# francesco-cal98/multimodal-idbn

Measured on AMD Instinct MI355X. Metric: CD-1 updates/sec (batch 64, 10000<->1500 RBM), higher is better.
Workload: dtype f32; 1 GPU; BASELINE configs[1] layer 1: RBM 10000<->1500 train_epoch, CD-1, batch 64 per GPU, fp32 master weights, lr 0.1 wd 1e-4 mom 0.5; global_batch=64, parallelism=dp1, arithmetic=bf16x3 split MFMA (fp32-exact products)

## Files before the change

include/imdbn_engine.h:

```cpp
#ifndef IMDBN_ENGINE_H
#define IMDBN_ENGINE_H

#include <stddef.h>
#include <stdint.h>

#ifdef __cplusplus
extern "C" {
#endif

#define IMDBN_ABI_VERSION 4

#define IMDBN_E_INVALID   (-1)
#define IMDBN_E_WORKSPACE (-2)
#define IMDBN_E_RNG       (-3)
#define IMDBN_E_NODEVICE  (-4)
#define IMDBN_E_UNSUPPORTED (-5)

#define IMDBN_PARITY_F32 0
#define IMDBN_FAST_BF16  1

#define IMDBN_RNG_PHILOX 0
#define IMDBN_RNG_REPLAY 1

#define IMDBN_MAX_GROUPS 4
// ... 52 lines not shown
    int32_t sample_h;
    int32_t sample_v;
    int32_t reclamp_negative;
    const float* next_data;
    int64_t ld_next;
    int32_t next_slot;
    int32_t data_slot;
    int32_t data_binary;
    int32_t next_binary;
    float*  fwd_out;
    int64_t ld_fwd;
} imdbn_cd_opts;

int    imdbn_version(void);
int    imdbn_last_error(char* buf, size_t n);
int    imdbn_device_info(int* cu_count, char* arch, size_t n);
size_t imdbn_ws_bytes(int V, int H, int B);
int    imdbn_set_tuning(int ksplit_up, int ksplit_down);
int    imdbn_set_option(const char* name, int value);
typedef struct imdbn_options imdbn_options;
imdbn_options* imdbn_options_create(void);
void   imdbn_options_destroy(imdbn_options* o);
int    imdbn_options_set(imdbn_options* o, const char* name, int value);
int    imdbn_use_options(const imdbn_options* o);
int    imdbn_profile_enable(int on);
int    imdbn_profile_read(double* total_ms, int* launches);
int    imdbn_debug_stamps(long long* out, int n);
int    imdbn_debug_ws_offset(int V, int H, int B, const char* name, size_t* offset);
enum { IMDBN_ROUTE_UP_FUSED = 0, IMDBN_ROUTE_UP_STREAM_BITS = 1, IMDBN_ROUTE_UP_STREAM_REAL = 2, IMDBN_ROUTE_UP_PARTIAL4 = 3,
       IMDBN_ROUTE_UP_PARTIAL = 4 };
enum { IMDBN_ROUTE_DOWN_K2_STREAM = 0, IMDBN_ROUTE_DOWN_FUSED = 1, IMDBN_ROUTE_DOWN_CHUNKS2 = 2, IMDBN_ROUTE_DOWN_CHUNKS4 = 3,
       IMDBN_ROUTE_DOWN_TILED = 4 };
int    imdbn_debug_last_route(int route[5]);

int imdbn_rng_advance(uint64_t* dev_offset, uint64_t n, imdbn_stream_t stream);

int imdbn_rbm_prop_up(const imdbn_rbm_desc* d, const float* v, int64_t ldv, int B, float T,
                      imdbn_rng* rng, float* out_prob, int64_t ldo, float* out_sample, int64_t lds,
                      void* ws, size_t ws_bytes, imdbn_stream_t stream);

int imdbn_rbm_forward(const imdbn_rbm_desc* d, const float* v, int64_t ldv, int B, int data_binary,
                      float* out_prob, int64_t ldo, void* ws, size_t ws_bytes, imdbn_stream_t stream);

int imdbn_rbm_free_energy(const imdbn_rbm_desc* d, const float* v, int64_t ldv, int B, float* out_F,
                          void* ws, size_t ws_bytes, imdbn_stream_t stream);

int imdbn_rbm_ais(const imdbn_rbm_desc* d, int M, int K, const float* betas, const float* base_vis_bias, imdbn_rng* rng,
                  double* logw, float* out_v, int64_t ldo, void* ws, size_t ws_bytes, imdbn_stream_t stream);

int imdbn_rbm_ais_groups(const imdbn_rbm_desc* d, int M, int K, const float* betas, const float* base_vis_bias, imdbn_rng* rng,
                         double* logw, float* out_v, int64_t ldo, void* ws, size_t ws_bytes, imdbn_stream_t stream);

int imdbn_rbm_reverse_ais(const imdbn_rbm_desc* d, const float* v, int64_t ldv, int R, int K, const float* betas,
                          const float* base_vis_bias, imdbn_rng* rng, double* logw, float* out_v, int64_t ldo,
                          void* ws, size_t ws_bytes, imdbn_stream_t stream);

int imdbn_rows_logmeanexp(const double* logw, int N, int M, double* out_lme, double* out_ess, imdbn_stream_t stream);

int imdbn_rbm_label_loglik(const imdbn_rbm_desc* d, const float* z, int64_t ldz, int N, int Dz, int K, const int32_t* gt,
                           double* out_joint, double* out_marg, void* ws, size_t ws_bytes, imdbn_stream_t stream);

int imdbn_rbm_label_step(const imdbn_rbm_desc* d, const float* z, int64_t ldz, int N, int Dz, int K, const int32_t* gt,
                         const imdbn_cd_opts* o, double* out_logp, float* scratch, void* ws, size_t ws_bytes, imdbn_stream_t stream);

int imdbn_rbm_pseudo_loglik(const imdbn_rbm_desc* d, const float* v, int64_t ldv, int N, double* out_pll, float* out_site, int64_t lds,
                            void* ws, size_t ws_bytes, imdbn_stream_t stream);
// ... 158 lines not shown
```

multimodal-idbn_amd/csrc/engine.hip:

```cpp
#include <hip/hip_runtime.h>

#include <algorithm>
#include <atomic>
#include <climits>
#include <cstdarg>
#include <cstdio>
#include <cstring>
#include <dlfcn.h>
#include <mutex>
#include <new>
#include <vector>

#include "../../include/imdbn_engine.h"
#include "kernels_ew.hpp"
#include "kernels_gemm.hpp"
#include "kernels_chain.hpp"
#include "kernels_stream.hpp"
#include "kernels_trace.hpp"
#include "kernels_knn.hpp"
#include "kernels_energy.hpp"
#include "kernels_metrics.hpp"
#include "kernels_ais.hpp"
#include "kernels_reverse_ais.hpp"
#include "kernels_bound.hpp"
// ... 480 lines not shown
    g_prof.calls = 0;
    return 0;
}

int imdbn_debug_stamps(long long* out, int n) {
    if (!out || n <= 0 || n > 4096 * 8) return fail(IMDBN_E_INVALID, "imdbn_debug_stamps: bad buffer");
    HIPCHK(hipDeviceSynchronize());
    HIPCHK(hipMemcpyFromSymbol(out, HIP_SYMBOL(g_stamps), sizeof(long long) * (size_t)n, 0, hipMemcpyDeviceToHost));
    static const std::vector<long long> zeros(4096 * 8, 0);
    HIPCHK(hipMemcpyToSymbol(HIP_SYMBOL(g_stamps), zeros.data(), sizeof(long long) * zeros.size(), 0, hipMemcpyHostToDevice));
    return 0;
}

int imdbn_debug_ws_offset(int V, int H, int B, const char* name, size_t* offset) {
    if (V <= 0 || H <= 0 || B <= 0 || !name || !offset) return fail(IMDBN_E_INVALID, "debug_ws_offset: bad argument");
    char* fake = reinterpret_cast<char*>((uintptr_t)1 << 30);
    const Layout L = make_layout(V, H, B, fake);
    const void* p = nullptr;
    if (!strcmp(name, "vis_bits0")) p = L.vis_bits[0]; else if (!strcmp(name, "vis_bits1")) p = L.vis_bits[1];
    else if (!strcmp(name, "hid_bits")) p = L.hid_bits; else if (!strcmp(name, "vis_tr0")) p = L.vis_tr[0];
    else if (!strcmp(name, "vis_tr1")) p = L.vis_tr[1]; else if (!strcmp(name, "hid_tr0")) p = L.hid_tr[0];
    else if (!strcmp(name, "hid_tr1")) p = L.hid_tr[1]; else if (!strcmp(name, "cs_hpos")) p = L.cs_hpos;
    else if (!strcmp(name, "cs_hneg")) p = L.cs_hneg; else if (!strcmp(name, "cs_vpos")) p = L.cs_vpos;
    else if (!strcmp(name, "cs_vneg")) p = L.cs_vneg; else if (!strcmp(name, "flags")) p = L.flags;
    else if (!strcmp(name, "partial")) p = L.partial; else if (!strcmp(name, "vis_rm1")) p = L.vis_rm[1];
    else return fail(IMDBN_E_INVALID, "debug_ws_offset: unknown buffer %s", name);
    *offset = (size_t)((const char*)p - fake);
    return 0;
}

int imdbn_debug_last_route(int route[5]) {
    if (!route) return fail(IMDBN_E_INVALID, "imdbn_debug_last_route: null buffer");
    route[0] = t_route.up; route[1] = t_route.up_general; route[2] = t_route.down; route[3] = t_route.down_general; route[4] = t_route.down_groups;
    return 0;
}

int imdbn_profile_read(double* total_ms, int* launches) {
    double tot = 0.0;
    for (size_t i = 0; i + 1 < g_prof.used; i += 2) {
        HIPCHK(hipEventSynchronize(g_prof.ev[i + 1]));
        float ms = 0.f;
        HIPCHK(hipEventElapsedTime(&ms, g_prof.ev[i], g_prof.ev[i + 1]));
        tot += ms;
    }
    if (total_ms) *total_ms = tot;
    if (launches) *launches = (int)(g_prof.used / 2);
    g_prof.used = 0;
    return 0;
}

__global__ void rng_advance_kernel(unsigned long long* p, unsigned long long n) { *p += n; }
int imdbn_rng_advance(uint64_t* dev_offset, uint64_t n, imdbn_stream_t stream) {
    if (!dev_offset) return fail(IMDBN_E_INVALID, "rng_advance: null counter");
    hipLaunchKernelGGL(rng_advance_kernel, dim3(1), dim3(1), 0, S(stream), (unsigned long long*)dev_offset, (unsigned long long)n);
    HIPCHK(hipGetLastError());
    return 0;
}

int imdbn_rbm_prop_up(const imdbn_rbm_desc* d, const float* v, int64_t ldv, int B, float T, imdbn_rng* rng,
                      float* out_prob, int64_t ldo, float* out_sample, int64_t lds, void* ws, size_t ws_bytes,
                      imdbn_stream_t stream) {
    CHK(check_desc(d, false));
    if (!v || !out_prob || ldv < d->V || ldo < d->H) return fail(IMDBN_E_INVALID, "prop_up: bad tensor argument");
    Ctx c(d, rng, S(stream));
    CHK(setup(c, B, ws, ws_bytes));
    FinishArgs f = new_finish();
// ... 485 lines not shown
    const Layout& L = c.L;
    const char* fb = fake + L.fb_off;
    if (((head_stride | planes_stride) & 255) || ((((uintptr_t)head) | ((uintptr_t)planes)) & 255) || planes_stride < L.fb_bytes ||
        head_stride < (size_t)((const char*)L.vis_tr[0] - fb))
        return fail(IMDBN_E_INVALID, "apply_factors: the gathered blocks must be 256-B aligned and at least %zu bytes apart", L.fb_bytes);
    auto at_h = [&](const void* layout_ptr, int rk) { return (const char*)head + ((const char*)layout_ptr - fb) + (size_t)rk * head_stride; };
    auto at_v = [&](const void* layout_ptr, int rk) { return (const char*)planes + ((const char*)layout_ptr - fb) + (size_t)rk * planes_stride; };
    AssocPlanesArgs f;
    memset(&f, 0, sizeof(f));
    f.W = d->W; f.Wm = d->W_m; f.ldw = d->ldw; f.V = L.V; f.H = L.H;
    f.vpos_terms = c.nw == 1 ? 1 : 0; f.vneg_terms = 1;
    f.vts = (int64_t)L.V * L.Bp; f.hts = (int64_t)L.H * L.Bp; f.Bp = L.Bp;
    f.lr = o->lr; f.mom = o->momentum; f.wd = o->weight_decay; f.n = (float)global_B;
    BiasArgs b = make_bias(c, o, o->sparsity != 0, (float)global_B, loss_out);
    b.hpos = (const float*)at_h(L.cs_hpos, 0); b.hneg = (const float*)at_h(L.cs_hneg, 0);
    b.vpos = (const float*)at_h(L.cs_vpos, 0); b.vneg = (const float*)at_h(L.cs_vneg, 0);
    b.loss_part = (const float*)at_h(L.loss_part, 0);
    b.R = n_ranks; b.rs = (int64_t)(head_stride / 4);
    BiasArgs bz;
    memset(&bz, 0, sizeof(bz));
    const int tpb = c.r.tpb, brows = k3_bias_rows(L);
    ProfBracket prof;
    CHK(prof.begin(c.s, true));
    if (n_ranks >= tune().min_rank_loop && !tune().no_rank_loop && f.vneg_terms == 1) {
        f.vpos = (const bf16_t*)at_v(L.vis_tr[0], 0); f.vpos_flag = (const int*)at_h(L.flags, 0);
        f.hpos = (const bf16_t*)at_h(L.hid_tr[0], 0);
        f.vneg = (const bf16_t*)at_v(L.vis_tr[1], 0); f.hneg = (const bf16_t*)at_h(L.hid_tr[1], 0);
        RankLoopArgs rl{n_ranks, (int64_t)(head_stride / 2), (int64_t)(planes_stride / 2)};
        const bool acc = tpb <= 4 && !tune().no_rank_acc;
        const auto k = c.ht == 3 ? (acc ? assoc_update_planes_ranks<3, true> : assoc_update_planes_ranks<3, false>)
                                 : (acc ? assoc_update_planes_ranks<1, true> : assoc_update_planes_ranks<1, false>);
        hipLaunchKernelGGL(k, k3_grid(c, brows), dim3(256), 0, c.s, f, rl, tpb, b, brows);
        HIPCHK(hipGetLastError());
        return prof.end(c.s);
    }
    for (int rk = 0; rk < n_ranks; ++rk) {
        f.vpos = (const bf16_t*)at_v(L.vis_tr[0], rk); f.vpos_flag = (const int*)at_h(L.flags, rk);
        f.hpos = (const bf16_t*)at_h(L.hid_tr[0], rk);
        f.vneg = (const bf16_t*)at_v(L.vis_tr[1], rk); f.hneg = (const bf16_t*)at_h(L.hid_tr[1], rk);
        const int br = (rk == n_ranks - 1) ? brows : 0;
        CHK(launch_k3_planes(c, 0, f, k3_pass(rk, n_ranks), br ? b : bz, br));
    }
    return prof.end(c.s);
}

int imdbn_rbm_apply_factors(const imdbn_rbm_desc* d, const void* gathered, int n_ranks, size_t rank_stride, int rows_per_rank,
                            int global_B, const imdbn_cd_opts* o, float* loss_out, imdbn_stream_t stream) {
    return apply_factors_impl(d, gathered, rank_stride, gathered, rank_stride, n_ranks, rows_per_rank, global_B, o, loss_out, stream);
}

int imdbn_rbm_apply_factors_wire(const imdbn_rbm_desc* d, const void* wire, size_t wire_stride, const void* planes, size_t planes_stride,
                                 int n_ranks, int rows_per_rank, int global_B, const imdbn_cd_opts* o, float* loss_out, imdbn_stream_t stream) {
    return apply_factors_impl(d, wire, wire_stride, planes, planes_stride, n_ranks, rows_per_rank, global_B, o, loss_out, stream);
}

int imdbn_rbm_apply_wire(const imdbn_rbm_desc* d, const void* wire, size_t wire_stride, int n_ranks, int rows_per_rank, int global_B,
                         int binary_data, void* planes, size_t planes_stride, const imdbn_cd_opts* o, float* loss_out, imdbn_stream_t stream) {
    CHK(check_desc(d, true));
    CHK(imdbn_rbm_unpack_factors(d->V, d->H, rows_per_rank, binary_data, wire, wire_stride, n_ranks, planes, planes_stride, 1, stream));
    return apply_factors_impl(d, wire, wire_stride, planes, planes_stride, n_ranks, rows_per_rank, global_B, o, loss_out, stream);
}

int imdbn_rbm_apply_delta(const imdbn_rbm_desc* d, const float* packed, int global_B, const imdbn_cd_opts* o,
                          float* loss_out, imdbn_stream_t stream) {
    CHK(check_desc(d, true));
    if (!packed || !o || global_B <= 0) return fail(IMDBN_E_INVALID, "apply_delta: bad argument");
// ... 739 lines not shown
```

multimodal-idbn_amd/csrc/host_layout.hpp:

```cpp
#pragma once

struct Tuning {
    int ks_up = 0, ks_down = 0;
    int no_fast_k3 = 0;
    int no_fast_k1 = 0;
    int no_fused_up = 0;
    int k4_rows = 0;
    int no_rank_loop = 0;
    int no_chain_kernel = 0;
    int no_rank_acc = 0;
    int min_rank_loop = 2;
    int no_prefetch = 0;
    int no_bits = 0;
    int down_tr = 0;
    int no_k1s = 0;
    int k1s_ks = 0;
    int no_k2s = 0;
    int k2s_tr = 0;
    int no_k1s_real = 0;
    int no_adaptive = 0;
    int k1s_lds_pad = 0;
    int no_chain_pair = 0;
    int no_down_tiled = 0;
    int no_down_chunks = 0;
    int k1s_force_na = 0;
};
Tuning g_defaults;
thread_local const Tuning* t_bound = nullptr;
inline const Tuning& tune() { return t_bound ? *t_bound : g_defaults; }
int g_dbg = 0;

enum OptKind { OPT_SET, OPT_FLAG, OPT_CLAMP, OPT_CHECKED };
struct Opt { const char* name; int Tuning::*knob; OptKind kind = OPT_SET; int lo = 0, hi = 0, step = 1; };
const Opt g_opts[] = {
    {"ksplit_up", &Tuning::ks_up, OPT_CLAMP, 0, INT_MAX}, {"ksplit_down", &Tuning::ks_down, OPT_CLAMP, 0, INT_MAX},
    {"k1s_ks", &Tuning::k1s_ks, OPT_CLAMP, 0, INT_MAX}, {"k1s_lds_pad", &Tuning::k1s_lds_pad, OPT_CLAMP, 0, 64 * 1024},
    {"down_rows", &Tuning::down_tr, OPT_CHECKED, 4, 32, 4}, {"k2s_rows", &Tuning::k2s_tr, OPT_CHECKED, 8, 48, 8},
    {"chain_rows", &Tuning::k4_rows, OPT_CHECKED, 0, 16, 1},
    {"generic_k3", &Tuning::no_fast_k3, OPT_FLAG}, {"generic_k1", &Tuning::no_fast_k1, OPT_FLAG}, {"no_fused_up", &Tuning::no_fused_up, OPT_FLAG},
    {"no_rank_loop", &Tuning::no_rank_loop}, {"no_rank_acc", &Tuning::no_rank_acc}, {"min_rank_loop", &Tuning::min_rank_loop},
    {"no_chain_kernel", &Tuning::no_chain_kernel}, {"no_chain_pair", &Tuning::no_chain_pair}, {"no_bits", &Tuning::no_bits},
    {"no_prefetch", &Tuning::no_prefetch}, {"no_adaptive", &Tuning::no_adaptive}, {"k1s_force_na", &Tuning::k1s_force_na},
    {"no_k1s", &Tuning::no_k1s}, {"no_k1s_real", &Tuning::no_k1s_real}, {"no_k2s", &Tuning::no_k2s},
    {"no_down_chunks", &Tuning::no_down_chunks}, {"no_down_tiled", &Tuning::no_down_tiled},
};

int set_opt(Tuning& t, const char* name, int value) {
    if (!name) return fail(IMDBN_E_INVALID, "null option name");
    if (!strcmp(name, "dbg")) { g_dbg = value; return 0; }
    for (const Opt& o : g_opts) {
        if (strcmp(name, o.name)) continue;
        if (o.kind == OPT_CHECKED && value != 0 && (value < o.lo || value > o.hi || value % o.step)) {
            if (o.step > 1) return fail(IMDBN_E_INVALID, "%s must be 0 or a multiple of %d in [%d, %d]", o.name, o.step, o.lo, o.hi);
            return fail(IMDBN_E_INVALID, "%s must be in [%d, %d]", o.name, o.lo, o.hi);
        }
        t.*o.knob = o.kind == OPT_FLAG ? (value != 0) : (o.kind == OPT_CLAMP ? std::max(o.lo, std::min(value, o.hi)) : value);
        return 0;
    }
    return fail(IMDBN_E_INVALID, "unknown option %s", name);
}

inline int rup(int x, int m) { return (x + m - 1) / m * m; }
inline int cdiv(int a, int b) { return (a + b - 1) / b; }

struct Split { int ks; int kchunk; };
Split plan_split(int Kpad, int n_tiles, int m_blocks, int forced, int cap) {
    int ks = forced;
    if (ks <= 0) {
        const int target = 768;
        ks = std::max(1, (int)((double)target / (double)(n_tiles * m_blocks) + 0.5));
    }
    ks = std::min(ks, cap);
    ks = std::min(ks, cdiv(Kpad, 64));
    ks = std::max(ks, 1);
    const int kchunk = rup(cdiv(Kpad, ks), 64);
    return {cdiv(Kpad, kchunk), kchunk};
}
// ... 153 lines not shown
    bool neg_rm;
    bool prefetch;
    bool next_on_k1;
    bool rides;
    bool adaptive_ok;
    bool adaptive_next;
    int tpb;
    int cd_k2_blocks;

    Up up(const OpIn& in, bool logits_only) const {
        if (up_fused) return Up::fused;
        if (!k1s || logits_only) return Up::partial;
        if (in.bits && (in.binary == 1 || in.binary == 2)) return Up::stream_bits;
        return (in.rm && k1s_real && (in.binary == 0 || (in.binary == 3 && in.bits && in.flag))) ? Up::stream_real : Up::partial;
    }
    bool data_bits(int data_binary) const { return k1s && data_binary != IMDBN_DATA_REAL; }
    bool data_needs_rm(int data_binary) const { return !(k1s && data_binary == IMDBN_DATA_BINARY); }
};

Route make_route(const imdbn_rbm_desc* d, const Layout& L) {
    const Tuning& t = tune();
    Route r{};
    r.vec4 = vec4_rows(d);
    r.up_fused = L.Vpad <= 1024 && !t.no_fused_up;
    r.k1s = r.vec4 && !t.no_k1s && !r.up_fused;
    r.k1s_real = r.k1s && !t.no_k1s_real;
    r.k2s = r.vec4 && !t.no_k2s;
    r.k2s_cd = r.k2s && !t.no_bits;
    r.vbits = d->n_groups == 0 && (r.k2s_cd || L.down_tr % 8 == 0);
    r.neg_rm = !(r.vbits && r.k1s);
    r.prefetch = r.vec4 && !t.no_prefetch;
    r.next_on_k1 = r.k2s_cd && r.vbits && r.k1s;
    r.rides = !r.k2s_cd || r.next_on_k1;
    r.tpb = std::max(1, cdiv(cdiv(L.H, 128) * cdiv(L.V, 128), std::max(cu_count(), 1)));
    r.adaptive_ok = L.k1s_kchunk <= 2048 && 2 * r.tpb * L.P <= 256 && cdiv(cdiv(L.V, 128), r.tpb) <= L.k1s_tiles * L.k1s_ks;
    r.adaptive_next = r.rides && !t.no_adaptive && r.k1s_real && r.adaptive_ok;
    r.cd_k2_blocks = cdiv(L.Vpad, r.k2s_cd ? L.k2s_tr : L.down_tr);
    return r;
}
```

multimodal-idbn_amd/csrc/host_update.hpp:

```cpp
#pragma once

struct Prof {
    bool on = false;
    std::vector<hipEvent_t> ev;
    size_t used = 0;
    unsigned calls = 0;
} g_prof;
struct ProfBracket {
    bool on = false;
    int begin(hipStream_t s, bool wanted) {
        on = wanted && g_prof.on && (g_prof.calls++ % 8 == 3) && g_prof.used + 2 <= g_prof.ev.size();
        if (on) HIPCHK(hipEventRecord(g_prof.ev[g_prof.used], s));
        return 0;
    }
    int end(hipStream_t s) {
        if (on) { HIPCHK(hipEventRecord(g_prof.ev[g_prof.used + 1], s)); g_prof.used += 2; }
        return 0;
    }
};

BiasArgs make_bias(Ctx& c, const imdbn_cd_opts* o, bool sparsity, float n, float* loss_out) {
    const Layout& L = c.L;
    BiasArgs b;
    memset(&b, 0, sizeof(b));
    b.hid_bias = c.d->hid_bias; b.hb_m = c.d->hb_m; b.H = L.H; b.hpos = L.cs_hpos; b.hneg = L.cs_hneg;
    b.vis_bias = c.d->vis_bias; b.vb_m = c.d->vb_m; b.V = L.V; b.vpos = L.cs_vpos; b.vneg = L.cs_vneg;
    b.P = L.P; b.lr = o->lr; b.mom = o->momentum; b.n = n;
    b.sparsity = sparsity ? 1 : 0; b.target = o->sparsity_target;
    b.loss_part = L.loss_part; b.n_loss = n_loss_used(c); b.loss_den = n * (float)L.V; b.loss_out = loss_out;
    return b;
}

BiasArgs make_pack(Ctx& c, float* packed) {
    const imdbn_rbm_desc* d = c.d;
    BiasArgs b;
    memset(&b, 0, sizeof(b));
    b.pack_tail = packed + (size_t)d->V * d->H; b.H = d->H; b.V = d->V;
    b.hpos = c.L.cs_hpos; b.hneg = c.L.cs_hneg; b.vpos = c.L.cs_vpos; b.vneg = c.L.cs_vneg; b.P = c.L.P;
    b.loss_part = c.L.loss_part; b.n_loss = n_loss_used(c);
    return b;
}

int launch_bias(Ctx& c, const BiasArgs& b) {
    hipLaunchKernelGGL(bias_update, dim3(cdiv(std::max(c.L.V, c.L.H), 256) + 1), dim3(256), 0, c.s, b);
    HIPCHK(hipGetLastError());
    return 0;
}

using K3Fn = decltype(&assoc_update_planes<0, 3, 0>);
const K3Fn k3_insts[2][2][4] = {
    {{assoc_update_planes<0, 1, 0>, assoc_update_planes<0, 1, 1>, assoc_update_planes<0, 1, 2>, assoc_update_planes<0, 1, 3>},
     {assoc_update_planes<0, 3, 0>, assoc_update_planes<0, 3, 1>, assoc_update_planes<0, 3, 2>, assoc_update_planes<0, 3, 3>}},
    {{assoc_update_planes<1, 1, 0>, assoc_update_planes<1, 1, 1>, assoc_update_planes<1, 1, 2>, assoc_update_planes<1, 1, 3>},
     {assoc_update_planes<1, 3, 0>, assoc_update_planes<1, 3, 1>, assoc_update_planes<1, 3, 2>, assoc_update_planes<1, 3, 3>}}};
int k3_pass(int i, int n) { return n == 1 ? 0 : (i == 0 ? 1 : (i == n - 1 ? 3 : 2)); }
int k3_bias_rows(const Layout& L) { return cdiv(L.H, 128) >= 2 ? 1 : 2; }
dim3 k3_grid(const Ctx& c, int br) { return dim3(cdiv(c.L.H, 128), cdiv(cdiv(c.L.V, 128), c.r.tpb) + br); }
int launch_k3_planes(Ctx& c, int mode_stats, const AssocPlanesArgs& f, int pass, const BiasArgs& bb, int br) {
    hipLaunchKernelGGL(k3_insts[mode_stats != 0][c.ht == 3][pass], k3_grid(c, br), dim3(256), 0, c.s, f, c.r.tpb, bb, br);
    HIPCHK(hipGetLastError());
    return 0;
}

int launch_assoc(Ctx& c, int mode_stats, const imdbn_cd_opts* o, int vpos_terms, const int* vpos_flag, int vneg_terms,
                 float n, float* delta, const BiasArgs* bias = nullptr) {
    const Layout& L = c.L;
    ProfBracket prof;
    CHK(prof.begin(c.s, !mode_stats));
    if (c.r.vec4 && (((uintptr_t)(mode_stats ? (const void*)delta : (const void*)c.d->W_m)) & 15) == 0 && !tune().no_fast_k3) {
        AssocPlanesArgs f;
        memset(&f, 0, sizeof(f));
        f.W = c.d->W; f.Wm = c.d->W_m; f.ldw = c.d->ldw; f.V = L.V; f.H = L.H;
        f.vpos = L.vis_tr[0]; f.vpos_flag = vpos_flag; f.vpos_terms = vpos_terms;
        f.hpos = L.hid_tr[0]; f.vneg = L.vis_tr[1]; f.vneg_terms = vneg_terms; f.hneg = L.hid_tr[1];
        f.vts = (int64_t)L.V * L.Bp; f.hts = (int64_t)L.H * L.Bp; f.Bp = L.Bp;
        f.lr = o->lr; f.mom = o->momentum; f.wd = o->weight_decay; f.n = n; f.delta = delta; f.dbg = (g_dbg & 512) ? 1 : 0;
        BiasArgs bz;
        memset(&bz, 0, sizeof(bz));
        const int nchunk = L.Bp / 64;
        for (int ch = 0; ch < nchunk; ++ch) {
            f.b0 = 64 * ch;
            CHK(launch_k3_planes(c, mode_stats, f, k3_pass(ch, nchunk), bias ? *bias : bz, (bias && ch == nchunk - 1) ? k3_bias_rows(L) : 0));
        }
        return prof.end(c.s);
    }
    AssocArgs a;
    memset(&a, 0, sizeof(a));
    a.W = c.d->W; a.Wm = c.d->W_m; a.ldw = c.d->ldw; a.V = L.V; a.H = L.H;
    a.vpos = L.vis_tr[0]; a.vpos_flag = vpos_flag; a.vpos_terms = vpos_terms;
    a.hpos = L.hid_tr[0]; a.hpos_terms = c.ht;
    a.vneg = L.vis_tr[1]; a.vneg_flag = vpos_flag; a.vneg_terms = vneg_terms;
    a.hneg = L.hid_tr[1]; a.hneg_terms = c.ht;
    a.vts = (int64_t)L.V * L.Bp; a.hts = (int64_t)L.H * L.Bp; a.Bp = L.Bp;
    a.lr = o->lr; a.mom = o->momentum; a.wd = o->weight_decay; a.n = n;
    a.delta = delta;
    hipLaunchKernelGGL(c.ht == 3 ? (mode_stats ? assoc_update<1, 3> : assoc_update<0, 3>) : (mode_stats ? assoc_update<1, 1> : assoc_update<0, 1>),
                       dim3(cdiv(L.H, 128), cdiv(L.V, 64)), dim3(256), 0, c.s, a);
    HIPCHK(hipGetLastError());
    CHK(prof.end(c.s));
    if (bias) CHK(launch_bias(c, *bias));
    return 0;
}
```

multimodal-idbn_amd/csrc/kernels_gemm.hpp:

```cpp
#pragma once
#include <type_traits>
#include "common.hpp"
#include "kernels_ew.hpp"

namespace imdbn {

template <int NW>
__device__ __forceinline__ void make_w_frags(const float (&wv)[8], uint4 (&frag)[NW]) {
    if constexpr (NW == 3) {
        uint32_t hi[8], mid[8], lo[8];
#pragma unroll
        for (int j = 0; j < 8; ++j) split3(wv[j], hi[j], mid[j], lo[j]);
        frag[0] = make_uint4(hi[0] | (hi[1] << 16), hi[2] | (hi[3] << 16), hi[4] | (hi[5] << 16), hi[6] | (hi[7] << 16));
        frag[1] = make_uint4(mid[0] | (mid[1] << 16), mid[2] | (mid[3] << 16), mid[4] | (mid[5] << 16), mid[6] | (mid[7] << 16));
        frag[2] = make_uint4(lo[0] | (lo[1] << 16), lo[2] | (lo[3] << 16), lo[4] | (lo[5] << 16), lo[6] | (lo[7] << 16));
    } else {
        uint32_t h[8];
#pragma unroll
        for (int j = 0; j < 8; ++j) h[j] = bf16_rne(wv[j]);
        frag[0] = make_uint4(h[0] | (h[1] << 16), h[2] | (h[3] << 16), h[4] | (h[5] << 16), h[6] | (h[7] << 16));
    }
}

__device__ __forceinline__ void reduce_store_tile(f32x16 (&acc)[2][2], float* __restrict__ slab ,
// ... 982 lines not shown
#pragma unroll
    for (int it = 0; it < 4; ++it) {
        if (it < n_my) {
            const int v0 = (tile0 + it) * 128;
#pragma unroll
            for (int reg = 0; reg < 16; ++reg) {
                const int row = min(v0 + 32 * w + mfma_row(reg, l), a.V - 1);
                const int64_t idx = (int64_t)row * a.ldw + colc;
                wc[reg] = *reinterpret_cast<const float4*>(a.W + idx);
                mc[reg] = *reinterpret_cast<const float4*>(a.Wm + idx);
            }
#pragma unroll
            for (int reg = 0; reg < 16; ++reg) {
                const int row = v0 + 32 * w + mfma_row(reg, l);
                if (row < a.V && cok) {
                    const float4 d = make_float4(acc[it][0][reg], acc[it][1][reg], acc[it][2][reg], acc[it][3][reg]);
                    const int64_t idx = (int64_t)row * a.ldw + h0 + 4 * r;
                    const float4 w0 = wc[reg];
                    float4 m = mc[reg];
                    const float gx = n_pow2 ? d.x * inv_n : d.x / a.n, gy = n_pow2 ? d.y * inv_n : d.y / a.n;
                    const float gz = n_pow2 ? d.z * inv_n : d.z / a.n, gw = n_pow2 ? d.w * inv_n : d.w / a.n;
                    m.x = m.x * a.mom; m.x = m.x + a.lr * (gx - a.wd * w0.x);
                    m.y = m.y * a.mom; m.y = m.y + a.lr * (gy - a.wd * w0.y);
                    m.z = m.z * a.mom; m.z = m.z + a.lr * (gz - a.wd * w0.z);
                    m.w = m.w * a.mom; m.w = m.w + a.lr * (gw - a.wd * w0.w);
                    *reinterpret_cast<float4*>(a.Wm + idx) = m;
                    *reinterpret_cast<float4*>(a.W + idx) = make_float4(w0.x + m.x, w0.y + m.y, w0.z + m.z, w0.w + m.w);
                }
            }
        }
    }
}

template <int HT, bool ACC>
__global__ __launch_bounds__(256, 1) void assoc_update_planes_ranks(const AssocPlanesArgs a, const RankLoopArgs rl, int tiles_per_block,
                                                                    const BiasArgs bias, int bias_rows) {
    __shared__ __attribute__((aligned(16))) char smem[K3_LDS_BYTES];
    if (bias_rows > 0 && (int)blockIdx.y >= (int)gridDim.y - bias_rows) {
        bias_work(bias, (blockIdx.y - (gridDim.y - bias_rows)) * gridDim.x + blockIdx.x, bias_rows * gridDim.x,
                  reinterpret_cast<double*>(smem));
        return;
    }
    int bx = blockIdx.x, by = blockIdx.y;
    {
        const int nbx = gridDim.x, nby = gridDim.y - bias_rows;
        int xa = 0;
        if (nbx % 2 == 0 && nby % 4 == 0) xa = 2; else if (nbx % 4 == 0 && nby % 2 == 0) xa = 4;
        else if (nby % 8 == 0) xa = 1; else if (nbx % 8 == 0) xa = 8;
        if (xa) {
            const int xc = 8 / xa, sa = nbx / xa, sc = nby / xc;
            const int p = blockIdx.y * nbx + blockIdx.x;
            const int xcd = p & 7, slot = p >> 3;
            bx = (xcd % xa) * sa + slot % sa;
            by = (xcd / xa) * sc + slot / sa;
        }
    }
    const int tile0 = by * tiles_per_block;
    const int ncbv = ((a.V + 15) / 16 * 16 + 63) / 64;
    int nap = a.vpos_terms;
    if (nap == 0) {
        nap = 1;
        for (int rk = 0; rk < rl.n_ranks; ++rk)
            nap = max(nap, operand_terms(a.vpos_flag + rk * (rl.stride_h / 2), ncbv, a.Bp / 8, (tile0 * 128) / 64, (tile0 + tiles_per_block) * 2, 0));
    }
    if constexpr (ACC) k3_body_ranks_acc<HT>(a, rl, smem, bx, by, tiles_per_block, nap, a.vneg_terms);
    else               k3_body_ranks<HT>(a, rl, smem, bx, by, tiles_per_block, nap, a.vneg_terms);
}

template <int MODE, int HT, int PASS>
__global__ __launch_bounds__(256, 1) void assoc_update_planes(const AssocPlanesArgs a, int tiles_per_block,
                                                              const BiasArgs bias, int bias_rows) {
    __shared__ __attribute__((aligned(16))) char smem[K3_LDS_BYTES];
    if (bias_rows > 0 && (int)blockIdx.y >= (int)gridDim.y - bias_rows) {
        bias_work(bias, (blockIdx.y - (gridDim.y - bias_rows)) * gridDim.x + blockIdx.x, bias_rows * gridDim.x,
                  reinterpret_cast<double*>(smem));
        return;
    }
    int bx = blockIdx.x, by = blockIdx.y;
    {
        const int nbx = gridDim.x, nby = gridDim.y - bias_rows;
        int xa = 0;
        if (nbx % 2 == 0 && nby % 4 == 0) xa = 2; else if (nbx % 4 == 0 && nby % 2 == 0) xa = 4;
        else if (nby % 8 == 0) xa = 1; else if (nbx % 8 == 0) xa = 8;
        if (xa) {
            const int xc = 8 / xa, sa = nbx / xa, sc = nby / xc;
            const int p = blockIdx.y * nbx + blockIdx.x;
            const int xcd = p & 7, slot = p >> 3;
            bx = (xcd % xa) * sa + slot % sa;
            by = (xcd / xa) * sc + slot / sa;
        }
    }
    const int tile0 = by * tiles_per_block;
    const int ncbv = ((a.V + 15) / 16 * 16 + 63) / 64;
    const int nap = operand_terms(a.vpos_flag, ncbv, a.Bp / 8, (tile0 * 128) / 64, (tile0 + tiles_per_block) * 2, a.vpos_terms);
    const int nan_ = a.vneg_terms;
    k3_body<MODE, HT, PASS>(a, smem, bx, by, tiles_per_block, nap, nan_);
}

template <int NW, int NA>
__device__ __forceinline__ void down_tiled_body(const float* __restrict__ W, int64_t ldw, int K, int N,
                                                const bf16_t* __restrict__ A, int64_t a_term_stride, int lda,
                                                const FinishArgs& fa, char* smem) {
    const int tid = threadIdx.x, w = __builtin_amdgcn_readfirstlane(tid >> 6), l = tid & 63, r = l & 31, hh = l >> 5;
    const int bx = blockIdx.x, bz = blockIdx.z;
    const int n0 = bx * 128, mb = bz * 64;
    const float* wrow = W + (int64_t)min(n0 + 32 * w + r, N - 1) * ldw;
    const int nblk = lda / 16, nslab = (nblk + 1) / 2;
    constexpr int SLOT = NA * 4096;
    const uint32_t ring_lds = __builtin_amdgcn_readfirstlane((uint32_t)(size_t)(__attribute__((address_space(3))) char*)smem);
    auto issue_a = [&](int s) __attribute__((always_inline)) {
#pragma unroll
        for (int q = 0; q < NA; ++q) {
            const int i = 4 * q + w;
            const int t = i >> 2, kb2 = (i >> 1) & 1, half = i & 1;
            const int kb = min(2 * s + kb2, nblk - 1);
            k3_dma16(A + t * a_term_stride + ((int64_t)kb * fa.Bp + mb + 32 * half) * 16 + 8 * l, ring_lds + (s & 1) * SLOT + i * 1024);
        }
    };
    float wv[16];
    auto load_w = [&](int s) __attribute__((always_inline)) {
#pragma unroll
        for (int kb2 = 0; kb2 < 2; ++kb2) {
            const int k0 = 16 * min(2 * s + kb2, nblk - 1) + 8 * hh;
            const float4 x0 = *reinterpret_cast<const float4*>(wrow + min(k0, K - 4));
            const float4 x1 = *reinterpret_cast<const float4*>(wrow + min(k0 + 4, K - 4));
            wv[8 * kb2 + 0] = x0.x; wv[8 * kb2 + 1] = x0.y; wv[8 * kb2 + 2] = x0.z; wv[8 * kb2 + 3] = x0.w;
            wv[8 * kb2 + 4] = x1.x; wv[8 * kb2 + 5] = x1.y; wv[8 * kb2 + 6] = x1.z; wv[8 * kb2 + 7] = x1.w;
        }
    };
// ... 89 lines not shown
```

multimodal-idbn_amd/imdbn/engine/native.py:

```python
from __future__ import annotations

import ctypes as C
import os

MAX_GROUPS = 4
ABI_VERSION = 4
PARITY_F32, FAST_BF16 = 0, 1
RNG_PHILOX, RNG_REPLAY = 0, 1
BOUND_ENTROPY, BOUND_LOGQ = 0, 1
DELTA_UP, DELTA_DOWN = 0, 1
DATA_UNKNOWN, DATA_BINARY, DATA_REAL = 0, 1, 2
ROUTE_UP = ("fused", "stream_bits", "stream_real", "partial4", "partial")
ROUTE_DOWN = ("k2_stream", "down_fused", "down_chunks2", "down_chunks4", "down_tiled")

_HERE = os.path.dirname(os.path.abspath(__file__))
LIB_PATH = os.path.normpath(os.path.join(_HERE, "..", "..", "lib", "libimdbn_hip.so"))


class RbmDesc(C.Structure):
    _fields_ = [
        ("W", C.c_void_p), ("ldw", C.c_int64),
        ("hid_bias", C.c_void_p), ("vis_bias", C.c_void_p),
        ("W_m", C.c_void_p), ("hb_m", C.c_void_p), ("vb_m", C.c_void_p),
        ("V", C.c_int32), ("H", C.c_int32), ("mode", C.c_int32), ("n_groups", C.c_int32),
# ... 39 lines not shown


class EnergyOut(C.Structure):
    _fields_ = [(n, C.c_void_p) for n in ("p_top1", "p_top2", "p_gt", "deltaF_pred", "l1", "k1", "steps_to_converge", "kstar", "predT",
                                          "margin_energy", "fe_top1", "fe_gap", "F", "y_final")]


class CrossMetricsOut(C.Structure):
    _fields_ = [(n, C.c_void_p) for n in ("pred", "gt", "p_pred", "p_true", "rank", "acc", "confusion", "class_sums")]


_P = C.c_void_p
_I64 = C.c_int64
_INT = C.c_int
_F = C.c_float
_SZ = C.c_size_t

SIGNATURES = {
    "imdbn_version": (_INT, []),
    "imdbn_last_error": (_INT, [C.c_char_p, _SZ]),
    "imdbn_device_info": (_INT, [C.POINTER(_INT), C.c_char_p, _SZ]),
    "imdbn_ws_bytes": (_SZ, [_INT, _INT, _INT]),
    "imdbn_set_tuning": (_INT, [_INT, _INT]),
    "imdbn_set_option": (_INT, [C.c_char_p, _INT]),
    "imdbn_options_create": (_P, []),
    "imdbn_options_destroy": (None, [_P]),
    "imdbn_options_set": (_INT, [_P, C.c_char_p, _INT]),
    "imdbn_use_options": (_INT, [_P]),
    "imdbn_profile_enable": (_INT, [_INT]),
    "imdbn_profile_read": (_INT, [C.POINTER(C.c_double), C.POINTER(_INT)]),
    "imdbn_debug_stamps": (_INT, [C.POINTER(C.c_longlong), _INT]),
    "imdbn_debug_ws_offset": (_INT, [_INT, _INT, _INT, C.c_char_p, C.POINTER(_SZ)]),
    "imdbn_debug_last_route": (_INT, [C.POINTER(_INT)]),
    "imdbn_rng_advance": (_INT, [_P, C.c_uint64, _P]),
    "imdbn_rbm_prop_up": (_INT, [C.POINTER(RbmDesc), _P, _I64, _INT, _F, C.POINTER(Rng), _P, _I64, _P, _I64, _P, _SZ, _P]),
    "imdbn_rbm_forward": (_INT, [C.POINTER(RbmDesc), _P, _I64, _INT, _INT, _P, _I64, _P, _SZ, _P]),
    "imdbn_rbm_free_energy": (_INT, [C.POINTER(RbmDesc), _P, _I64, _INT, _P, _P, _SZ, _P]),
    "imdbn_rbm_ais": (_INT, [C.POINTER(RbmDesc), _INT, _INT, C.POINTER(_F), _P, C.POINTER(Rng), _P, _P, _I64, _P, _SZ, _P]),
    "imdbn_rbm_ais_groups": (_INT, [C.POINTER(RbmDesc), _INT, _INT, C.POINTER(_F), _P, C.POINTER(Rng), _P, _P, _I64, _P, _SZ, _P]),
    "imdbn_rbm_reverse_ais": (_INT, [C.POINTER(RbmDesc), _P, _I64, _INT, _INT, C.POINTER(_F), _P, C.POINTER(Rng), _P, _P, _I64, _P, _SZ, _P]),
    "imdbn_rows_logmeanexp": (_INT, [_P, _INT, _INT, _P, _P, _P]),
    "imdbn_rbm_label_loglik": (_INT, [C.POINTER(RbmDesc), _P, _I64, _INT, _INT, _INT, _P, _P, _P, _P, _SZ, _P]),
    "imdbn_rbm_label_step": (_INT, [C.POINTER(RbmDesc), _P, _I64, _INT, _INT, _INT, _P, C.POINTER(CdOpts), _P, _P, _P, _SZ, _P]),
    "imdbn_rbm_pseudo_loglik": (_INT, [C.POINTER(RbmDesc), _P, _I64, _INT, _P, _P, _I64, _P, _SZ, _P]),
    "imdbn_rbm_bound_step": (_INT, [C.POINTER(RbmDesc), _P, _I64, _INT, _INT, C.POINTER(Rng), _P, _P, _I64, _P, _SZ, _P]),
    "imdbn_rbm_prop_down": (_INT, [C.POINTER(RbmDesc), _P, _I64, _INT, _F, _INT, _P, _I64, _P, _SZ, _P]),
    "imdbn_rbm_sample_visible": (_INT, [C.POINTER(RbmDesc), _P, _I64, _INT, C.POINTER(Rng), _P, _I64, _P]),
    "imdbn_rbm_gibbs_step": (_INT, [C.POINTER(RbmDesc), _P, _I64, _INT, _INT, _INT, C.POINTER(Rng), _P, _P, _P, _P, _P, _SZ, _P]),
    "imdbn_rbm_cd_step": (_INT, [C.POINTER(RbmDesc), _P, _I64, _INT, C.POINTER(CdOpts), C.POINTER(Rng), _P, _P, _SZ, _P]),
    "imdbn_rbm_pcd_step": (_INT, [C.POINTER(RbmDesc), _P, _I64, _INT, _P, _I64, C.POINTER(CdOpts), C.POINTER(Rng), _P, _P, _SZ, _P]),
    "imdbn_centered_scratch_floats": (_SZ, [_INT, _INT]),
    "imdbn_rbm_centered_step": (_INT, [C.POINTER(RbmDesc), _P, _I64, _INT, _P, _I64, C.POINTER(CdOpts), C.POINTER(Rng), _P, _P, C.c_float, _INT,
                                       _P, _P, _P, _SZ, _P]),
    "imdbn_rbm_delta_step": (_INT, [C.POINTER(RbmDesc), _INT, _P, _I64, _P, _I64, _INT, C.POINTER(CdOpts), _P, _P, _SZ, _P]),
    "imdbn_rbm_pt_sweep": (_INT, [C.POINTER(RbmDesc), _P, _I64, _INT, _INT, C.POINTER(_F), _INT, C.POINTER(Rng), _P, _P, _P, _SZ, _P]),
    "imdbn_packed_delta_floats": (_SZ, [_INT, _INT]),
    "imdbn_rbm_prefetch_ok": (_INT, [C.POINTER(RbmDesc), _INT]),
    "imdbn_factor_compact_bytes": (_INT, [_INT, _INT, _INT, _INT, C.POINTER(_SZ)]),
    "imdbn_rbm_pack_factors": (_INT, [_INT, _INT, _INT, _INT, _P, _P, _P]),
    "imdbn_rbm_unpack_factors": (_INT, [_INT, _INT, _INT, _INT, _P, _SZ, _INT, _P, _SZ, _INT, _P]),
    "imdbn_rbm_cd_factors_wire": (_INT, [C.POINTER(RbmDesc), _P, _I64, _INT, C.POINTER(CdOpts), C.POINTER(Rng), _INT, _P, _P, _SZ, _P]),
    "imdbn_rbm_apply_wire": (_INT, [C.POINTER(RbmDesc), _P, _SZ, _INT, _INT, _INT, _INT, _P, _SZ, C.POINTER(CdOpts), _P, _P]),
    "imdbn_rbm_apply_factors_wire": (_INT, [C.POINTER(RbmDesc), _P, _SZ, _P, _SZ, _INT, _INT, _INT, C.POINTER(CdOpts), _P, _P]),
    "imdbn_rbm_cd_stats": (_INT, [C.POINTER(RbmDesc), _P, _I64, _INT, C.POINTER(CdOpts), C.POINTER(Rng), _P, _P, _SZ, _P]),
    "imdbn_rbm_apply_delta": (_INT, [C.POINTER(RbmDesc), _P, _INT, C.POINTER(CdOpts), _P, _P]),
    "imdbn_factor_block": (_INT, [_INT, _INT, _INT, C.POINTER(_SZ), C.POINTER(_SZ)]),
# ... 59 lines not shown
```

Before: 10420 updates/s.

## Add specialized single-chunk binary weight-update kernel with register-prefetched W/momentum

Adds an assoc_update_bin kernel, used when there is a single 64-row batch chunk with one positive and one negative bf16 operand term. It prefetches the next tile's W and momentum rows into registers, split around the MFMA phase, and double-buffers the visible slices through async LDS DMA, so global memory traffic overlaps compute. The epilogue is fused with a power-of-two reciprocal fast path. It also adds a k3_tpb override, an opt-out flag and a debug record of which update kernel ran, at the cost of high register pressure from the doubled float4 arrays.

```diff
diff --git a/include/imdbn_engine.h b/include/imdbn_engine.h
--- a/include/imdbn_engine.h
+++ b/include/imdbn_engine.h
@@ -108,6 +108,8 @@
 enum { IMDBN_ROUTE_DOWN_K2_STREAM = 0, IMDBN_ROUTE_DOWN_FUSED = 1, IMDBN_ROUTE_DOWN_CHUNKS2 = 2, IMDBN_ROUTE_DOWN_CHUNKS4 = 3,
        IMDBN_ROUTE_DOWN_TILED = 4 };
 int    imdbn_debug_last_route(int route[5]);
+enum { IMDBN_UPDATE_GENERIC = 0, IMDBN_UPDATE_PLANES = 1, IMDBN_UPDATE_BIN = 2, IMDBN_UPDATE_RANKS = 3 };
+int    imdbn_debug_last_update(int rec[2]);
 
 int imdbn_rng_advance(uint64_t* dev_offset, uint64_t n, imdbn_stream_t stream);
 
diff --git a/multimodal-idbn_amd/csrc/engine.hip b/multimodal-idbn_amd/csrc/engine.hip
--- a/multimodal-idbn_amd/csrc/engine.hip
+++ b/multimodal-idbn_amd/csrc/engine.hip
@@ -536,6 +536,12 @@
 int imdbn_debug_last_route(int route[5]) {
     if (!route) return fail(IMDBN_E_INVALID, "imdbn_debug_last_route: null buffer");
     route[0] = t_route.up; route[1] = t_route.up_general; route[2] = t_route.down; route[3] = t_route.down_general; route[4] = t_route.down_groups;
+    return 0;
+}
+
+int imdbn_debug_last_update(int rec[2]) {
+    if (!rec) return fail(IMDBN_E_INVALID, "imdbn_debug_last_update: null buffer");
+    rec[0] = t_update.kernel; rec[1] = t_update.tpb;
     return 0;
 }
 
@@ -1087,6 +1093,7 @@
                                  : (acc ? assoc_update_planes_ranks<1, true> : assoc_update_planes_ranks<1, false>);
         hipLaunchKernelGGL(k, k3_grid(c, brows), dim3(256), 0, c.s, f, rl, tpb, b, brows);
         HIPCHK(hipGetLastError());
+        ran_update(IMDBN_UPDATE_RANKS, tpb);
         return prof.end(c.s);
     }
     for (int rk = 0; rk < n_ranks; ++rk) {
diff --git a/multimodal-idbn_amd/csrc/host_layout.hpp b/multimodal-idbn_amd/csrc/host_layout.hpp
--- a/multimodal-idbn_amd/csrc/host_layout.hpp
+++ b/multimodal-idbn_amd/csrc/host_layout.hpp
@@ -22,6 +22,8 @@
     int k1s_lds_pad = 0;
     int no_chain_pair = 0;
     int no_down_tiled = 0;
+    int no_update_bin = 0;
+    int k3_tpb = 0;
     int no_down_chunks = 0;
     int k1s_force_na = 0;
 };
@@ -43,6 +45,7 @@
     {"no_prefetch", &Tuning::no_prefetch}, {"no_adaptive", &Tuning::no_adaptive}, {"k1s_force_na", &Tuning::k1s_force_na},
     {"no_k1s", &Tuning::no_k1s}, {"no_k1s_real", &Tuning::no_k1s_real}, {"no_k2s", &Tuning::no_k2s},
     {"no_down_chunks", &Tuning::no_down_chunks}, {"no_down_tiled", &Tuning::no_down_tiled},
+    {"no_update_bin", &Tuning::no_update_bin}, {"k3_tpb", &Tuning::k3_tpb, OPT_CLAMP, 0, 64},
 };
 
 int set_opt(Tuning& t, const char* name, int value) {
@@ -262,7 +265,7 @@
     r.prefetch = r.vec4 && !t.no_prefetch;
     r.next_on_k1 = r.k2s_cd && r.vbits && r.k1s;
     r.rides = !r.k2s_cd || r.next_on_k1;
-    r.tpb = std::max(1, cdiv(cdiv(L.H, 128) * cdiv(L.V, 128), std::max(cu_count(), 1)));
+    r.tpb = t.k3_tpb > 0 ? t.k3_tpb : std::max(1, cdiv(cdiv(L.H, 128) * cdiv(L.V, 128), std::max(cu_count(), 1)));
     r.adaptive_ok = L.k1s_kchunk <= 2048 && 2 * r.tpb * L.P <= 256 && cdiv(cdiv(L.V, 128), r.tpb) <= L.k1s_tiles * L.k1s_ks;
     r.adaptive_next = r.rides && !t.no_adaptive && r.k1s_real && r.adaptive_ok;
     r.cd_k2_blocks = cdiv(L.Vpad, r.k2s_cd ? L.k2s_tr : L.down_tr);
diff --git a/multimodal-idbn_amd/csrc/host_update.hpp b/multimodal-idbn_amd/csrc/host_update.hpp
--- a/multimodal-idbn_amd/csrc/host_update.hpp
+++ b/multimodal-idbn_amd/csrc/host_update.hpp
@@ -47,6 +47,10 @@
     return 0;
 }
 
+struct UpdateRec { int kernel = -1, tpb = 0; };
+thread_local UpdateRec t_update;
+inline void ran_update(int kernel, int tpb) { t_update.kernel = kernel; t_update.tpb = tpb; }
+
 using K3Fn = decltype(&assoc_update_planes<0, 3, 0>);
 const K3Fn k3_insts[2][2][4] = {
     {{assoc_update_planes<0, 1, 0>, assoc_update_planes<0, 1, 1>, assoc_update_planes<0, 1, 2>, assoc_update_planes<0, 1, 3>},
@@ -56,9 +60,11 @@
 int k3_pass(int i, int n) { return n == 1 ? 0 : (i == 0 ? 1 : (i == n - 1 ? 3 : 2)); }
 int k3_bias_rows(const Layout& L) { return cdiv(L.H, 128) >= 2 ? 1 : 2; }
 dim3 k3_grid(const Ctx& c, int br) { return dim3(cdiv(c.L.H, 128), cdiv(cdiv(c.L.V, 128), c.r.tpb) + br); }
-int launch_k3_planes(Ctx& c, int mode_stats, const AssocPlanesArgs& f, int pass, const BiasArgs& bb, int br) {
-    hipLaunchKernelGGL(k3_insts[mode_stats != 0][c.ht == 3][pass], k3_grid(c, br), dim3(256), 0, c.s, f, c.r.tpb, bb, br);
+int launch_k3_planes(Ctx& c, int mode_stats, const AssocPlanesArgs& f, int pass, const BiasArgs& bb, int br, bool bin = false) {
+    const K3Fn k = bin ? (c.ht == 3 ? assoc_update_bin<3> : assoc_update_bin<1>) : k3_insts[mode_stats != 0][c.ht == 3][pass];
+    hipLaunchKernelGGL(k, k3_grid(c, br), dim3(256), 0, c.s, f, c.r.tpb, bb, br);
     HIPCHK(hipGetLastError());
+    ran_update(bin ? IMDBN_UPDATE_BIN : IMDBN_UPDATE_PLANES, c.r.tpb);
     return 0;
 }
 
@@ -78,9 +84,11 @@
         BiasArgs bz;
         memset(&bz, 0, sizeof(bz));
         const int nchunk = L.Bp / 64;
+        const bool bin = !mode_stats && nchunk == 1 && vneg_terms == 1 && (vpos_terms == 1 || (vpos_terms == 0 && vpos_flag)) &&
+                         !tune().no_update_bin;
         for (int ch = 0; ch < nchunk; ++ch) {
             f.b0 = 64 * ch;
-            CHK(launch_k3_planes(c, mode_stats, f, k3_pass(ch, nchunk), bias ? *bias : bz, (bias && ch == nchunk - 1) ? k3_bias_rows(L) : 0));
+            CHK(launch_k3_planes(c, mode_stats, f, k3_pass(ch, nchunk), bias ? *bias : bz, (bias && ch == nchunk - 1) ? k3_bias_rows(L) : 0, bin));
         }
         return prof.end(c.s);
     }
@@ -97,6 +105,7 @@
     hipLaunchKernelGGL(c.ht == 3 ? (mode_stats ? assoc_update<1, 3> : assoc_update<0, 3>) : (mode_stats ? assoc_update<1, 1> : assoc_update<0, 1>),
                        dim3(cdiv(L.H, 128), cdiv(L.V, 64)), dim3(256), 0, c.s, a);
     HIPCHK(hipGetLastError());
+    ran_update(IMDBN_UPDATE_GENERIC, 0);
     CHK(prof.end(c.s));
     if (bias) CHK(launch_bias(c, *bias));
     return 0;
diff --git a/multimodal-idbn_amd/csrc/kernels_gemm.hpp b/multimodal-idbn_amd/csrc/kernels_gemm.hpp
--- a/multimodal-idbn_amd/csrc/kernels_gemm.hpp
+++ b/multimodal-idbn_amd/csrc/kernels_gemm.hpp
@@ -1038,29 +1038,36 @@
     }
 }
 
+__device__ __forceinline__ bool k3_bias_block(const BiasArgs& bias, int bias_rows, char* smem) {
+    if (bias_rows > 0 && (int)blockIdx.y >= (int)gridDim.y - bias_rows) {
+        bias_work(bias, (blockIdx.y - (gridDim.y - bias_rows)) * gridDim.x + blockIdx.x, bias_rows * gridDim.x,
+                  reinterpret_cast<double*>(smem));
+        return true;
+    }
+    return false;
+}
+__device__ __forceinline__ void k3_block_map(int bias_rows, int& bx, int& by) {
+    bx = blockIdx.x; by = blockIdx.y;
+    const int nbx = gridDim.x, nby = gridDim.y - bias_rows;
+    int xa = 0;
+    if (nbx % 2 == 0 && nby % 4 == 0) xa = 2; else if (nbx % 4 == 0 && nby % 2 == 0) xa = 4;
+    else if (nby % 8 == 0) xa = 1; else if (nbx % 8 == 0) xa = 8;
+    if (xa) {
+        const int xc = 8 / xa, sa = nbx / xa, sc = nby / xc;
+        const int p = blockIdx.y * nbx + blockIdx.x;
+        const int xcd = p & 7, slot = p >> 3;
+        bx = (xcd % xa) * sa + slot % sa;
+        by = (xcd / xa) * sc + slot / sa;
+    }
+}
+
 template <int HT, bool ACC>
 __global__ __launch_bounds__(256, 1) void assoc_update_planes_ranks(const AssocPlanesArgs a, const RankLoopArgs rl, int tiles_per_block,
                                                                     const BiasArgs bias, int bias_rows) {
     __shared__ __attribute__((aligned(16))) char smem[K3_LDS_BYTES];
-    if (bias_rows > 0 && (int)blockIdx.y >= (int)gridDim.y - bias_rows) {
-        bias_work(bias, (blockIdx.y - (gridDim.y - bias_rows)) * gridDim.x + blockIdx.x, bias_rows * gridDim.x,
-                  reinterpret_cast<double*>(smem));
-        return;
-    }
-    int bx = blockIdx.x, by = blockIdx.y;
-    {
-        const int nbx = gridDim.x, nby = gridDim.y - bias_rows;
-        int xa = 0;
-        if (nbx % 2 == 0 && nby % 4 == 0) xa = 2; else if (nbx % 4 == 0 && nby % 2 == 0) xa = 4;
-        else if (nby % 8 == 0) xa = 1; else if (nbx % 8 == 0) xa = 8;
-        if (xa) {
-            const int xc = 8 / xa, sa = nbx / xa, sc = nby / xc;
-            const int p = blockIdx.y * nbx + blockIdx.x;
-            const int xcd = p & 7, slot = p >> 3;
-            bx = (xcd % xa) * sa + slot % sa;
-            by = (xcd / xa) * sc + slot / sa;
-        }
-    }
+    if (k3_bias_block(bias, bias_rows, smem)) return;
+    int bx, by;
+    k3_block_map(bias_rows, bx, by);
     const int tile0 = by * tiles_per_block;
     const int ncbv = ((a.V + 15) / 16 * 16 + 63) / 64;
     int nap = a.vpos_terms;
@@ -1077,30 +1084,148 @@
 __global__ __launch_bounds__(256, 1) void assoc_update_planes(const AssocPlanesArgs a, int tiles_per_block,
                                                               const BiasArgs bias, int bias_rows) {
     __shared__ __attribute__((aligned(16))) char smem[K3_LDS_BYTES];
-    if (bias_rows > 0 && (int)blockIdx.y >= (int)gridDim.y - bias_rows) {
-        bias_work(bias, (blockIdx.y - (gridDim.y - bias_rows)) * gridDim.x + blockIdx.x, bias_rows * gridDim.x,
-                  reinterpret_cast<double*>(smem));
-        return;
-    }
-    int bx = blockIdx.x, by = blockIdx.y;
-    {
-        const int nbx = gridDim.x, nby = gridDim.y - bias_rows;
-        int xa = 0;
-        if (nbx % 2 == 0 && nby % 4 == 0) xa = 2; else if (nbx % 4 == 0 && nby % 2 == 0) xa = 4;
-        else if (nby % 8 == 0) xa = 1; else if (nbx % 8 == 0) xa = 8;
-        if (xa) {
-            const int xc = 8 / xa, sa = nbx / xa, sc = nby / xc;
-            const int p = blockIdx.y * nbx + blockIdx.x;
-            const int xcd = p & 7, slot = p >> 3;
-            bx = (xcd % xa) * sa + slot % sa;
-            by = (xcd / xa) * sc + slot / sa;
-        }
-    }
+    if (k3_bias_block(bias, bias_rows, smem)) return;
+    int bx, by;
+    k3_block_map(bias_rows, bx, by);
     const int tile0 = by * tiles_per_block;
     const int ncbv = ((a.V + 15) / 16 * 16 + 63) / 64;
     const int nap = operand_terms(a.vpos_flag, ncbv, a.Bp / 8, (tile0 * 128) / 64, (tile0 + tiles_per_block) * 2, a.vpos_terms);
     const int nan_ = a.vneg_terms;
     k3_body<MODE, HT, PASS>(a, smem, bx, by, tiles_per_block, nap, nan_);
+}
+
+constexpr int K3B_TOP = 12;
+static_assert(32 + 2 * K3B_TOP <= 63, "the vmcnt field holds 6 bits");
+
+template <int HT>
+__device__ __forceinline__ void k3_body_bin(const AssocPlanesArgs& a, char* smem, int bx, int by, int tiles_per_block) {
+    const int tid = threadIdx.x, w = tid >> 6, l = tid & 63, r = l & 31, kh = l >> 5;
+    const int h0 = bx * 128;
+    const int tile0 = by * tiles_per_block;
+    const int n_vtiles = (a.V + 127) / 128;
+    const int n_my = min(tiles_per_block, n_vtiles - tile0);
+    const int colc = min(h0 + 4 * r, a.H - 4);
+    const bool cok = (h0 + 4 * r) < a.H;
+    const bool n_pow2 = (__float_as_uint(a.n) & 0x7fffffu) == 0u;
+    const float inv_n = 1.0f / a.n;
+
+    char* sHp = smem;
+    char* sHn = smem + 3 * K3_PLANE;
+    char* sV = smem + K3_VIS0 + w * (4 * K3_SLICE);
+    const uint32_t sV_lds = __builtin_amdgcn_readfirstlane((uint32_t)(size_t)(__attribute__((address_space(3))) char*)sV);
+
+    auto load_rows = [&](auto r0_tag, auto r1_tag, float4 (&wo)[16], float4 (&mo)[16], int v0, bool valid) {
+#pragma unroll
+        for (int reg = decltype(r0_tag)::value; reg < decltype(r1_tag)::value; ++reg) {
+            const int row = valid ? min(v0 + 32 * w + mfma_row(reg, l), a.V - 1) : tile0 * 128;
+            const int64_t idx = (int64_t)row * a.ldw + colc;
+            wo[reg] = *reinterpret_cast<const float4*>(a.W + idx);
+            mo[reg] = *reinterpret_cast<const float4*>(a.Wm + idx);
+        }
+    };
+    auto dma_slices = [&](int buf, int v0w) {
+#pragma unroll
+        for (int ph = 0; ph < 2; ++ph)
+#pragma unroll
+            for (int q = 0; q < 4; ++q) {
+                const int i = l + 64 * q, row = i >> 3, c = (i & 7) ^ ((row >> 1) & 7);
+                k3_dma16((ph ? a.vneg : a.vpos) + (int64_t)min(v0w + row, a.V - 1) * a.Bp + a.b0 + 8 * c,
+                         sV_lds + (2 * buf + ph) * K3_SLICE + q * 1024);
+            }
+    };
+    using I0 = std::integral_constant<int, 0>;
+    using IT = std::integral_constant<int, K3B_TOP>;
+    using IE = std::integral_constant<int, 16>;
+
+    float4 wA[16], mA[16], wB[16], mB[16];
+    const bool st = a.dbg != 0;
+    const int sblk = by * gridDim.x + bx;
+    stamp(st, sblk, 0);
+    const uint32_t sH_lds = __builtin_amdgcn_readfirstlane((uint32_t)(size_t)(__attribute__((address_space(3))) char*)smem);
+#pragma unroll
+    for (int ph = 0; ph < 2; ++ph)
+#pragma unroll
+        for (int tb = 0; tb < HT; ++tb)
+#pragma unroll
+            for (int jj = 0; jj < 4; ++jj) {
+                const int j = 4 * w + jj, i = 64 * j + l, lrow = i >> 3, pos = i & 7;
+                const int row = 4 * (lrow & 31) + (lrow >> 5), c = pos ^ ((lrow >> 1) & 7);
+                const bf16_t* src = (ph ? a.hneg : a.hpos) + tb * a.hts + (int64_t)min(h0 + row, a.H - 1) * a.Bp + a.b0 + 8 * c;
+                k3_dma16(src, sH_lds + (3 * ph + tb) * K3_PLANE + j * 1024);
+            }
+    dma_slices(0, tile0 * 128 + 32 * w);
+    __builtin_amdgcn_sched_barrier(0);
+    load_rows(I0{}, IE{}, wA, mA, tile0 * 128, true);
+    __builtin_amdgcn_sched_barrier(0);
+    asm volatile("s_waitcnt vmcnt(32)" ::: "memory");
+    __syncthreads();
+    stamp(st, sblk, 1);
+
+    auto tile = [&](int it, auto buf_tag, float4 (&wc)[16], float4 (&mc)[16], float4 (&wn)[16], float4 (&mn)[16]) {
+        constexpr int BUF = decltype(buf_tag)::value;
+        const int v0 = (tile0 + it) * 128;
+        const bool more = it + 1 < n_my;
+        load_rows(I0{}, IT{}, wn, mn, v0 + 128, more);
+        __builtin_amdgcn_sched_barrier(0);
+        asm volatile("s_waitcnt vmcnt(%0)" :: "i"(32 + 2 * K3B_TOP) : "memory");
+        f32x16 acc[4];
+#pragma unroll
+        for (int t = 0; t < 4; ++t)
+#pragma unroll
+            for (int i = 0; i < 16; ++i) acc[t][i] = 0.f;
+        k3_mfma_wave<HT>(acc, sHp, sV + (2 * BUF) * K3_SLICE, r, kh);
+        k3_mfma_wave<HT>(acc, sHn, sV + (2 * BUF + 1) * K3_SLICE, r, kh);
+        asm volatile("s_waitcnt lgkmcnt(0)" ::: "memory");
+        __builtin_amdgcn_sched_barrier(0);
+        load_rows(IT{}, IE{}, wn, mn, v0 + 128, more);
+        __builtin_amdgcn_sched_barrier(0);
+        if (more) dma_slices(BUF ^ 1, v0 + 128 + 32 * w);
+        __builtin_amdgcn_sched_barrier(0);
+        auto epilogue = [&](auto pow2_tag) {
+            constexpr bool POW2 = decltype(pow2_tag)::value;
+#pragma unroll
+            for (int reg = 0; reg < 16; ++reg) {
+                const int row = v0 + 32 * w + mfma_row(reg, l);
+                if (row < a.V && cok) {
+                    const float4 d = make_float4(acc[0][reg], acc[1][reg], acc[2][reg], acc[3][reg]);
+                    const int64_t idx = (int64_t)row * a.ldw + h0 + 4 * r;
+                    const float4 w0 = wc[reg];
+                    float4 m = mc[reg];
+                    const float gx = POW2 ? d.x * inv_n : d.x / a.n, gy = POW2 ? d.y * inv_n : d.y / a.n;
+                    const float gz = POW2 ? d.z * inv_n : d.z / a.n, gw = POW2 ? d.w * inv_n : d.w / a.n;
+                    m.x = m.x * a.mom; m.x = m.x + a.lr * (gx - a.wd * w0.x);
+                    m.y = m.y * a.mom; m.y = m.y + a.lr * (gy - a.wd * w0.y);
+                    m.z = m.z * a.mom; m.z = m.z + a.lr * (gz - a.wd * w0.z);
+                    m.w = m.w * a.mom; m.w = m.w + a.lr * (gw - a.wd * w0.w);
+                    *reinterpret_cast<float4*>(a.Wm + idx) = m;
+                    *reinterpret_cast<float4*>(a.W + idx) = make_float4(w0.x + m.x, w0.y + m.y, w0.z + m.z, w0.w + m.w);
+                }
+            }
+        };
+        if (n_pow2) epilogue(std::true_type{}); else epilogue(std::false_type{});
+        stamp(st, sblk, 2 + it);
+    };
+    for (int it = 0; it < n_my; it += 2) {
+        tile(it, std::integral_constant<int, 0>{}, wA, mA, wB, mB);
+        if (it + 1 < n_my) tile(it + 1, std::integral_constant<int, 1>{}, wB, mB, wA, mA);
+    }
+}
+
+template <int HT>
+__global__ __launch_bounds__(256, 1) void assoc_update_bin(const AssocPlanesArgs a, int tiles_per_block,
+                                                           const BiasArgs bias, int bias_rows) {
+    __shared__ __attribute__((aligned(16))) char smem[K3_LDS_BYTES];
+    if (k3_bias_block(bias, bias_rows, smem)) return;
+    int bx, by;
+    k3_block_map(bias_rows, bx, by);
+    const int tile0 = by * tiles_per_block;
+    const int ncbv = ((a.V + 15) / 16 * 16 + 63) / 64;
+    const int nap = operand_terms(a.vpos_flag, ncbv, a.Bp / 8, (tile0 * 128) / 64, (tile0 + tiles_per_block) * 2, a.vpos_terms);
+    if (nap != 1) {
+        k3_body<0, HT, 0>(a, smem, bx, by, tiles_per_block, nap, a.vneg_terms);
+        return;
+    }
+    k3_body_bin<HT>(a, smem, bx, by, tiles_per_block);
 }
 
 template <int NW, int NA>
diff --git a/multimodal-idbn_amd/imdbn/engine/native.py b/multimodal-idbn_amd/imdbn/engine/native.py
--- a/multimodal-idbn_amd/imdbn/engine/native.py
+++ b/multimodal-idbn_amd/imdbn/engine/native.py
@@ -95,6 +95,7 @@
     "imdbn_debug_stamps": (_INT, [C.POINTER(C.c_longlong), _INT]),
     "imdbn_debug_ws_offset": (_INT, [_INT, _INT, _INT, C.c_char_p, C.POINTER(_SZ)]),
     "imdbn_debug_last_route": (_INT, [C.POINTER(_INT)]),
+    "imdbn_debug_last_update": (_INT, [C.POINTER(_INT)]),
     "imdbn_rng_advance": (_INT, [_P, C.c_uint64, _P]),
     "imdbn_rbm_prop_up": (_INT, [C.POINTER(RbmDesc), _P, _I64, _INT, _F, C.POINTER(Rng), _P, _I64, _P, _I64, _P, _SZ, _P]),
     "imdbn_rbm_forward": (_INT, [C.POINTER(RbmDesc), _P, _I64, _INT, _INT, _P, _I64, _P, _SZ, _P]),
```

New measurement: 10720 updates/s, median of 6. +2.8%, better.
